# 001camellia/Speech-Imagery-EEG

Hardware: AMD Instinct MI355X
Metric: epochs/sec (B=256, C=122, T=1000) IGN 3-class (higher is better)
Workload: dtype f32

## Files before the change

speech-imagery-eeg_amd/csrc/ign_clconv_x6.hip:

```cpp
#include "ign_clconv.h"

typedef __bf16 bf16x8 __attribute__((ext_vector_type(8)));
constexpr int X6_PITCH = KC + 8;
constexpr int X6_PLANE = TM * X6_PITCH;
constexpr int X6_BLOCK = 3 * TN * KC;

typedef float f32x2 __attribute__((ext_vector_type(2)));
typedef __bf16 bf16x2 __attribute__((ext_vector_type(2)));
__device__ __forceinline__ void split3_pair(f32x2 v, bf16x2& x0, bf16x2& x1, bf16x2& x2) {
    x0 = __builtin_convertvector(v, bf16x2);
    f32x2 r = v - __builtin_convertvector(x0, f32x2);
    x1 = __builtin_convertvector(r, bf16x2);
    r -= __builtin_convertvector(x1, f32x2);
    x2 = __builtin_convertvector(r, bf16x2);
}
template <int V>
__device__ __forceinline__ void split3_store(const float (&t)[V], __bf16* d, int plane);
template <>
__device__ __forceinline__ void split3_store<1>(const float (&t)[1], __bf16* d, int plane);
__device__ __forceinline__ void split3(float v, __bf16& x0, __bf16& x1, __bf16& x2) {
    x0 = (__bf16)v;
    float r = v - (float)x0;
    x1 = (__bf16)r;
    r -= (float)x1;
    x2 = (__bf16)r;
}
template <>
__device__ __forceinline__ void split3_store<1>(const float (&t)[1], __bf16* d, int plane) {
    __bf16 x0, x1, x2;
    split3(t[0], x0, x1, x2);
    d[0] = x0; d[plane] = x1; d[2 * plane] = x2;
}
template <>
__device__ __forceinline__ void split3_store<2>(const float (&t)[2], __bf16* d, int plane) {
    bf16x2 x0, x1, x2;
    split3_pair(f32x2{t[0], t[1]}, x0, x1, x2);
    *reinterpret_cast<bf16x2*>(d) = x0;
    *reinterpret_cast<bf16x2*>(d + plane) = x1;
    *reinterpret_cast<bf16x2*>(d + 2 * plane) = x2;
}
template <>
__device__ __forceinline__ void split3_store<4>(const float (&t)[4], __bf16* d, int plane) {
    typedef __bf16 bf16x4 __attribute__((ext_vector_type(4)));
    bf16x2 a0, a1, a2, b0, b1, b2;
    split3_pair(f32x2{t[0], t[1]}, a0, a1, a2);
    split3_pair(f32x2{t[2], t[3]}, b0, b1, b2);
    *reinterpret_cast<bf16x4*>(d) = __builtin_shufflevector(a0, b0, 0, 1, 2, 3);
    *reinterpret_cast<bf16x4*>(d + plane) = __builtin_shufflevector(a1, b1, 0, 1, 2, 3);
    *reinterpret_cast<bf16x4*>(d + 2 * plane) = __builtin_shufflevector(a2, b2, 0, 1, 2, 3);
}

typedef _Float16 f16x2 __attribute__((ext_vector_type(2)));
typedef _Float16 f16x4 __attribute__((ext_vector_type(4)));
typedef _Float16 f16x8 __attribute__((ext_vector_type(8)));
__device__ __forceinline__ void split2h_pair(f32x2 v, f16x2& x0, f16x2& x1) {
    x0 = __builtin_convertvector(v, f16x2);
    x1 = __builtin_convertvector(v - __builtin_convertvector(x0, f32x2), f16x2);
}
template <int V>
__device__ __forceinline__ void split2h_store(const float (&t)[V], __bf16* d, int plane) {
    _Float16* dh = reinterpret_cast<_Float16*>(d);
    if constexpr (V == 1) {
        const _Float16 x0 = (_Float16)t[0];
        dh[0] = x0; dh[plane] = (_Float16)(t[0] - (float)x0);
    } else if constexpr (V == 2) {
        f16x2 x0, x1;
        split2h_pair(f32x2{t[0], t[1]}, x0, x1);
        *reinterpret_cast<f16x2*>(dh) = x0;
        *reinterpret_cast<f16x2*>(dh + plane) = x1;
    } else {
        f16x2 a0, a1, b0, b1;
        split2h_pair(f32x2{t[0], t[1]}, a0, a1);
        split2h_pair(f32x2{t[2], t[3]}, b0, b1);
        *reinterpret_cast<f16x4*>(dh) = __builtin_shufflevector(a0, b0, 0, 1, 2, 3);
        *reinterpret_cast<f16x4*>(dh + plane) = __builtin_shufflevector(a1, b1, 0, 1, 2, 3);
    }
}

template <int V, int NP>
__device__ __forceinline__ void split_store(const float (&t)[V], __bf16* d, int plane) {
    if constexpr (NP == 3) {
        split3_store<V>(t, d, plane);
    } else if constexpr (NP == 2) {
        split2h_store<V>(t, d, plane);
    } else if constexpr (V == 1) {
        d[0] = (__bf16)t[0];
    } else if constexpr (V == 2) {
        *reinterpret_cast<bf16x2*>(d) = __builtin_convertvector(f32x2{t[0], t[1]}, bf16x2);
    } else {
        typedef __bf16 bf16x4 __attribute__((ext_vector_type(4)));
        const bf16x2 a = __builtin_convertvector(f32x2{t[0], t[1]}, bf16x2), b = __builtin_convertvector(f32x2{t[2], t[3]}, bf16x2);
        *reinterpret_cast<bf16x4*>(d) = __builtin_shufflevector(a, b, 0, 1, 2, 3);
    }
}

template <int NP>
__device__ __forceinline__ f32x16 mfma16(const bf16x8& a, const bf16x8& b, const f32x16& c) {
    if constexpr (NP == 2)
        return __builtin_amdgcn_mfma_f32_32x32x16_f16(__builtin_bit_cast(f16x8, a), __builtin_bit_cast(f16x8, b), c, 0, 0, 0);
    else
        return __builtin_amdgcn_mfma_f32_32x32x16_bf16(a, b, c, 0, 0, 0);
}

#ifndef IGN_H3_WAVES
#define IGN_H3_WAVES 3
#endif
constexpr int X6T_SPAN = TM + 15;
constexpr int X6T_APLANE = X6T_SPAN * X6_PITCH;

template <int NP> struct X6tLds {
    static constexpr int NPL = (NP == 2) ? 2 : 3;
    static constexpr int ABUF = NPL * X6T_APLANE, BBUF = NPL * X6_PLANE;
    static constexpr size_t BYTES = (size_t)2 * (ABUF + BBUF) * sizeof(unsigned short);
};
template <int NP, int EPI> struct X6tWaves { static constexpr int N = (NP == 2 && EPI == EPI_BIAS_STATS) ? IGN_H3_WAVES : 2; };
template <int V, bool PRO, int EPI, int NP>
__global__ void __launch_bounds__(256, (X6tWaves<NP, EPI>::N)) clconv_x6t_kernel(const ConvX6Args ca) {
    const GemmNTArgs& a = ca.g;
    constexpr int VPR = KC / V;
    constexpr int APASS = (X6T_SPAN * VPR + 255) / 256;
    constexpr int X6T_ABUF = X6tLds<NP>::ABUF, X6T_BBUF = X6tLds<NP>::BBUF;
    extern __shared__ __attribute__((aligned(16))) unsigned short smem16[];
    __bf16* Abuf = reinterpret_cast<__bf16*>(smem16);
    __bf16* Bbuf = Abuf + 2 * X6T_ABUF;

    const int nwg = a.mtiles * a.ntiles;
    int lid = blockIdx.x;
    {
        const int per = nwg / 8;
        if (lid < per * 8) lid = (lid & 7) * per + (lid >> 3);
    }
    const int mt = lid / a.ntiles, nt = lid - mt * a.ntiles;
    const int bi = mt / ca.tps, tt = mt - bi * ca.tps;
    const int t0 = tt * TM, n0 = nt * TN;
    const int tid = threadIdx.x, lane = tid & 63, wave = tid >> 6;
    const int l31 = lane & 31, h = lane >> 5;
    const int wm = wave & 1, wn = wave >> 1;
    const int span = TM + ca.k - 1;
    const int nvec = span * VPR;

    const float* abase = a.A + (long long)bi * ca.sample_pitch;
    const int brw = tid >> 1, bh = tid & 1;
    const unsigned short* bsrc = a.B3 + (size_t)nt * (size_t)(ca.cp / KC) * ca.k * X6_BLOCK + (size_t)brw * KC + 8 * bh;
    constexpr size_t bplane = (size_t)TN * KC;

    f32x16 acc[2][2];
#pragma unroll
    for (int i = 0; i < 2; ++i)
#pragma unroll
        for (int j = 0; j < 2; ++j)
#pragma unroll
            for (int r = 0; r < 16; ++r) acc[i][j][r] = 0.f;

    float ra[APASS][V];
    float pa[V], pb[V];
    bool a_ok = false;
    uint4 rb00, rb01 = {}, rb02 = {}, rb10, rb11 = {}, rb12 = {};
    const int ncc = ca.cp / KC;
    const int nstep = ncc * ca.k;

    const float sa = (NP == 2) ? ign_pow2_scale(ca.bound_a) : 1.f;
    const float osc = (NP == 2) ? 1.f / (sa * ign_pow2_scale(ca.bound_b)) : 1.f;
    auto aload = [&](int cc) {
        const int ch = cc * KC + (tid % VPR) * V;
        a_ok = ch < ca.cin;
        if (PRO && a_ok) {
            vload<V>(pa, a.pro_a + ch); vload<V>(pb, a.pro_b + ch);
            if constexpr (NP == 2) {
#pragma unroll
                for (int v = 0; v < V; ++v) { pa[v] *= sa; pb[v] *= sa; }
            }
        }
#pragma unroll
        for (int p = 0; p < APASS; ++p) {
            const int idx = tid + p * 256;
            const int row = idx / VPR;
            if (a_ok && idx < nvec) vload<V>(ra[p], abase + (long long)min(t0 + row, ca.rows_in - 1) * ca.cin + ch);
            else {
#pragma unroll
                for (int v = 0; v < V; ++v) ra[p][v] = 0.f;
            }
        }
    };
    auto astore = [&](int buf) {
        __bf16* st = Abuf + buf * X6T_ABUF;
#pragma unroll
        for (int p = 0; p < APASS; ++p) {
            const int idx = tid + p * 256;
            if (idx < nvec) {
                const int row = idx / VPR, q = idx - row * VPR;
                float tv[V];
#pragma unroll
                for (int v = 0; v < V; ++v) {
                    tv[v] = ra[p][v];
                    if (PRO && a_ok) tv[v] = fmaxf(fmaf(pa[v], tv[v], pb[v]), 0.f);
                    else if (NP == 2) tv[v] *= sa;
                }
                split_store<V, NP>(tv, st + row * X6_PITCH + q * V, X6T_APLANE);
            }
        }
    };
    auto boff = [&](int st) {
        st = min(st, nstep - 1);
        return (size_t)st * X6_BLOCK;
    };
    auto bstore = [&](int buf, const uint4& r0, const uint4& r1, const uint4& r2) {
        __bf16* st = Bbuf + buf * X6T_BBUF + brw * X6_PITCH + 8 * bh;
        *reinterpret_cast<uint4*>(st) = r0;
        if constexpr (NP >= 2) *reinterpret_cast<uint4*>(st + X6_PLANE) = r1;
        if constexpr (NP == 3) *reinterpret_cast<uint4*>(st + 2 * X6_PLANE) = r2;
    };
#define IGN_BLOAD(r0, r1, r2, st)                                                                       \
    do {                                                                                                \
        const size_t off_ = boff(st);                                                                   \
        r0 = *reinterpret_cast<const uint4*>(bsrc + off_);                                              \
        if constexpr (NP >= 2) r1 = *reinterpret_cast<const uint4*>(bsrc + bplane + off_);              \
        if constexpr (NP == 3) r2 = *reinterpret_cast<const uint4*>(bsrc + 2 * bplane + off_);          \
    } while (0)

    aload(0);
    IGN_BLOAD(rb00, rb01, rb02, 0);
    IGN_BLOAD(rb10, rb11, rb12, 1);
    astore(0);
    bstore(0, rb00, rb01, rb02);
    __syncthreads();

    int cc = 0, j = 0;
    auto body = [&](int step, bool odd) {
        if (odd) IGN_BLOAD(rb10, rb11, rb12, step + 2);
        else IGN_BLOAD(rb00, rb01, rb02, step + 2);
        const bool next_span = cc + 1 < ncc;
        if (j == 0 && next_span) aload(cc + 1);
        const __bf16* As = Abuf + (cc & 1) * X6T_ABUF + (wm * 64 + l31 + j) * X6_PITCH + 8 * h;
        const __bf16* Bs = Bbuf + (step & 1) * X6T_BBUF + (wn * 64 + l31) * X6_PITCH + 8 * h;
        bf16x8 af[2][NP], bf[2][NP];
#pragma unroll
        for (int i = 0; i < 2; ++i)
#pragma unroll
            for (int pl = 0; pl < NP; ++pl) {
                af[i][pl] = *reinterpret_cast<const bf16x8*>(As + pl * X6T_APLANE + i * 32 * X6_PITCH);
                bf[i][pl] = *reinterpret_cast<const bf16x8*>(Bs + pl * X6_PLANE + i * 32 * X6_PITCH);
            }
        __builtin_amdgcn_sched_barrier(0);
#define IGN_X6(pa_, pb_)                                                                                   \
        acc[0][0] = mfma16<NP>(af[0][pa_], bf[0][pb_], acc[0][0]);                                         \
        acc[0][1] = mfma16<NP>(af[0][pa_], bf[1][pb_], acc[0][1]);                                         \
        acc[1][0] = mfma16<NP>(af[1][pa_], bf[0][pb_], acc[1][0]);                                         \
        acc[1][1] = mfma16<NP>(af[1][pa_], bf[1][pb_], acc[1][1]);
        if constexpr (NP == 3) { IGN_X6(2, 0) IGN_X6(0, 2) IGN_X6(1, 1) IGN_X6(1, 0) IGN_X6(0, 1) }
        if constexpr (NP == 2) { IGN_X6(1, 0) IGN_X6(0, 1) }
        IGN_X6(0, 0)
#undef IGN_X6
        __builtin_amdgcn_sched_barrier(0);
        if (odd) bstore((step + 1) & 1, rb00, rb01, rb02);
        else bstore((step + 1) & 1, rb10, rb11, rb12);
        if (j + 1 == ca.k) {
            if (next_span) astore((cc + 1) & 1);
            j = 0; ++cc;
        } else {
            ++j;
        }
        __syncthreads();
    };
    for (int step = 0; step < nstep; step += 2) {
        body(step, false);
        if (step + 1 < nstep) body(step + 1, true);
    }
#undef IGN_BLOAD
    const int m0 = bi * ca.trows + t0;
    nt_epilogue<EPI, NP == 2>(a, acc, reinterpret_cast<float*>(smem16), mt, m0, n0, bi * ca.trows + min(ca.trows, t0 + TM), osc);
}

#ifndef IGN_H3W_WAVES
#define IGN_H3W_WAVES 2
#endif
template <int NP> struct X6wLds {
    static constexpr int NPL = NP == 3 ? 3 : (NP == 2 ? 2 : 1);
    static constexpr int ABUF = NPL * TM * X6_PITCH;
    static constexpr int BBUF = 2 * NPL * X6_PLANE;
    static constexpr size_t BYTES = (size_t)2 * (ABUF + BBUF) * sizeof(unsigned short);
    static constexpr int WAVES = NP == 2 ? IGN_H3W_WAVES : 2;
};

template <int NP, int EPI = EPI_BIAS_STATS>
__global__ void __launch_bounds__(512, X6wLds<NP>::WAVES) clconv_x6w_kernel(const ConvX6Args ca) {
    const GemmNTArgs& a = ca.g;
    extern __shared__ __attribute__((aligned(16))) unsigned short smem16[];
    constexpr int X6W_ABUF = X6wLds<NP>::ABUF, X6W_BBUF = X6wLds<NP>::BBUF, NPL = X6wLds<NP>::NPL;
    __bf16* Abuf = reinterpret_cast<__bf16*>(smem16);
    __bf16* Bbuf = Abuf + 2 * X6W_ABUF;
    constexpr int APLANE = TM * X6_PITCH;

    const int ntw = a.N / 256;
    const int nwg = a.mtiles * ntw;
    int lid = blockIdx.x;
    {
        const int per = nwg / 8;
        if (lid < per * 8) lid = (lid & 7) * per + (lid >> 3);
    }
    const int mt = lid / ntw, nw = lid - mt * ntw;
    const int m0 = mt * TM, n0 = nw * 256;
    const int tid = threadIdx.x, lane = tid & 63, wave = tid >> 6;
    const int l31 = lane & 31, h = lane >> 5;
    const int wm = wave & 1, wn = wave >> 1;
    const int ncc = ca.cp / KC;

    f32x16 acc[2][2];
#pragma unroll
    for (int i = 0; i < 2; ++i)
#pragma unroll
        for (int j = 0; j < 2; ++j)
#pragma unroll
            for (int r = 0; r < 16; ++r) acc[i][j][r] = 0.f;

    const int arow = tid >> 2, ach = (tid & 3) * 4;
    const float* ap = a.A + (long long)min(m0 + arow, a.M - 1) * ca.cin + ach;
    float ra0[4], ra1[4];
    const int bt = tid >> 8, brw = (tid & 255) >> 1, bh = tid & 1;
    const unsigned short* bsrc = a.B3 + (size_t)(2 * nw + bt) * (size_t)ncc * X6_BLOCK + (size_t)brw * KC + 8 * bh;
    constexpr size_t bplane = (size_t)TN * KC;
    uint4 rb00, rb01 = {}, rb02 = {}, rb10, rb11 = {}, rb12 = {};

    const float sa = (NP == 2) ? ign_pow2_scale(ca.bound_a) : 1.f;
    const float osc = (NP == 2) ? 1.f / (sa * ign_pow2_scale(ca.bound_b)) : 1.f;
#define IGN_ALOADW(ra_, cc_)                                                                 \
    do {                                                                                     \
        const int c_ = min((cc_), ncc - 1);                                                  \
        if (c_ * KC + ach < ca.cin) vload<4>(ra_, ap + c_ * KC);           \
        else ra_[0] = ra_[1] = ra_[2] = ra_[3] = 0.f;                                        \
    } while (0)
    auto astore = [&](int buf, const float (&r)[4]) {
        if constexpr (NP == 2) {
            const float rs[4] = {r[0] * sa, r[1] * sa, r[2] * sa, r[3] * sa};
            split_store<4, NP>(rs, Abuf + buf * X6W_ABUF + arow * X6_PITCH + ach, APLANE);
        } else {
            split_store<4, NP>(r, Abuf + buf * X6W_ABUF + arow * X6_PITCH + ach, APLANE);
        }
    };
    auto bstore = [&](int buf, const uint4& r0, const uint4& r1, const uint4& r2) {
        __bf16* st = Bbuf + buf * X6W_BBUF + bt * NPL * X6_PLANE + brw * X6_PITCH + 8 * bh;
        *reinterpret_cast<uint4*>(st) = r0;
        if constexpr (NP >= 2) *reinterpret_cast<uint4*>(st + X6_PLANE) = r1;
        if constexpr (NP == 3) *reinterpret_cast<uint4*>(st + 2 * X6_PLANE) = r2;
    };
#define IGN_BLOADW(r0, r1, r2, st)                                                                      \
    do {                                                                                                \
        const size_t off_ = (size_t)min((st), ncc - 1) * X6_BLOCK;                                      \
        r0 = *reinterpret_cast<const uint4*>(bsrc + off_);                                              \
        if constexpr (NP >= 2) r1 = *reinterpret_cast<const uint4*>(bsrc + bplane + off_);              \
        if constexpr (NP == 3) r2 = *reinterpret_cast<const uint4*>(bsrc + 2 * bplane + off_);          \
    } while (0)

    IGN_ALOADW(ra0, 0);
    IGN_BLOADW(rb00, rb01, rb02, 0);
    IGN_ALOADW(ra1, 1);
    IGN_BLOADW(rb10, rb11, rb12, 1);
    astore(0, ra0);
    bstore(0, rb00, rb01, rb02);
    __syncthreads();

    const bool late = wave >= 4;
    auto mm = [&](int step) {
        const __bf16* As = Abuf + (step & 1) * X6W_ABUF + (wm * 64 + l31) * X6_PITCH + 8 * h;
        const __bf16* Bs = Bbuf + (step & 1) * X6W_BBUF + (wn >> 1) * NPL * X6_PLANE + ((wn & 1) * 64 + l31) * X6_PITCH + 8 * h;
        bf16x8 af[2][NP], bf[2][NP];
#pragma unroll
        for (int i = 0; i < 2; ++i)
#pragma unroll
            for (int pl = 0; pl < NP; ++pl) {
                af[i][pl] = *reinterpret_cast<const bf16x8*>(As + pl * APLANE + i * 32 * X6_PITCH);
                bf[i][pl] = *reinterpret_cast<const bf16x8*>(Bs + pl * X6_PLANE + i * 32 * X6_PITCH);
            }
        __builtin_amdgcn_sched_barrier(0);
#define IGN_X6(pa_, pb_)                                                                                   \
        acc[0][0] = mfma16<NP>(af[0][pa_], bf[0][pb_], acc[0][0]);                                         \
        acc[0][1] = mfma16<NP>(af[0][pa_], bf[1][pb_], acc[0][1]);                                         \
        acc[1][0] = mfma16<NP>(af[1][pa_], bf[0][pb_], acc[1][0]);                                         \
        acc[1][1] = mfma16<NP>(af[1][pa_], bf[1][pb_], acc[1][1]);
        if constexpr (NP == 3) { IGN_X6(2, 0) IGN_X6(0, 2) IGN_X6(1, 1) }
        if constexpr (NP >= 2) { IGN_X6(1, 0) IGN_X6(0, 1) }
        IGN_X6(0, 0)
#undef IGN_X6
        __builtin_amdgcn_sched_barrier(0);
    };
    auto body = [&](int step, bool odd) {
        if (odd) { IGN_BLOADW(rb10, rb11, rb12, step + 2); IGN_ALOADW(ra1, step + 2); }
        else { IGN_BLOADW(rb00, rb01, rb02, step + 2); IGN_ALOADW(ra0, step + 2); }
        const bool next = step + 1 < ncc;
        auto st = [&]() {
            if (odd) { bstore((step + 1) & 1, rb00, rb01, rb02); if (next) astore((step + 1) & 1, ra0); }
            else { bstore((step + 1) & 1, rb10, rb11, rb12); if (next) astore((step + 1) & 1, ra1); }
            __builtin_amdgcn_sched_barrier(0);
        };
        if (late) { st(); mm(step); } else { mm(step); st(); }
        __syncthreads();
    };
    for (int step = 0; step < ncc; step += 2) {
        body(step, false);
        if (step + 1 < ncc) body(step + 1, true);
    }
#undef IGN_BLOADW
#undef IGN_ALOADW
    float s1[2] = {0.f, 0.f}, s2[2] = {0.f, 0.f};
    const int m_lim = a.M;
    if (m0 + TM <= m_lim) nt_epilogue_body<EPI, true, NP == 2>(a, acc, s1, s2, m0, n0, m_lim, osc);
    else nt_epilogue_body<EPI, false, NP == 2>(a, acc, s1, s2, m0, n0, m_lim, osc);
}

__device__ __forceinline__ void pack_weights_x3t_body(const float* __restrict__ w, unsigned short* __restrict__ wt3,
                                                      unsigned short* __restrict__ wd3, int Co, int Ci, int k, int Cip, int Cop,
                                                      long long i, const float* __restrict__ bound = nullptr) {
    const long long nf = (long long)((Co + TN - 1) / TN) * (Cip / KC) * k * (TN * KC);
    const long long nd = wd3 ? (long long)((Ci + TN - 1) / TN) * (Cop / KC) * k * (TN * KC) : 0;
    const bool fwd = i < nf;
    if (!fwd && i >= nf + nd) return;
    const long long e = fwd ? i : i - nf;
    const int q = (int)(e % KC);
    long long t = e / KC;
    const int row = (int)(t % TN);
    t /= TN;
    const int j = (int)(t % k);
    t /= k;
    const int ncc = (fwd ? Cip : Cop) / KC;
// ... 214 lines not shown
    float* out = a.part + (long long)split * a.Co * a.k * a.Ci;
    const int ci = ci0 + wci * 32 + l31;
    if (ci < a.Ci) {
#pragma unroll
        for (int j = 0; j < KT; ++j)
#pragma unroll
            for (int r = 0; r < 16; ++r) {
                const int co = co0 + wco * 32 + acc_row16(r, h);
                if (co < a.Co) out[((long long)co * a.k + j) * a.Ci + ci] = (NP == 2) ? acc[j][r] * osc : acc[j][r];
            }
    }
}

constexpr int W1_PITCH = 128 + 32;
constexpr int W1_PLANE = 16 * W1_PITCH;

struct Wgrad1Args {
    const float* dy; const float* x; float* part;
    float* part_b;
    long long M;
    int Ci, Co, nunits, nsplit, citiles, ntiles;
    const float* bound_dy; const float* bound_x;
};

template <int NP>
__global__ void __launch_bounds__(256, (NP == 2 ? IGN_H3_WAVES : 2)) clconv_wgrad_x6_k1_kernel(const Wgrad1Args a) {
    extern __shared__ __attribute__((aligned(16))) unsigned short smem16[];
    __bf16* smem = reinterpret_cast<__bf16*>(smem16);
    constexpr int NPL = (NP == 2) ? 2 : 3;
    constexpr int W1_STAGE = 2 * NPL * W1_PLANE;
    const int xcd = blockIdx.x & 7, seq = blockIdx.x >> 3;
    const int tile = seq % a.ntiles;
    const int split = (seq / a.ntiles) * 8 + xcd;
    if (split >= a.nsplit) return;
    const int cot = tile / a.citiles, cit = tile - cot * a.citiles;
    const int co0 = cot * 128, ci0 = cit * 128;
    const int per = (a.nunits + a.nsplit - 1) / a.nsplit;
    const int u_begin = split * per, u_end = min(a.nunits, u_begin + per);

    const int tid = threadIdx.x, lane = tid & 63, wave = tid >> 6;
    const int l31 = lane & 31, h = lane >> 5;
    const int wco = wave & 1, wci = wave >> 1;

    const int sr = tid >> 5, sc = (tid & 31) * 4;
    const bool d_ok = co0 + sc < a.Co, x_ok = ci0 + sc < a.Ci;
    const float* dyp = a.dy + co0 + sc;
    const float* xp = a.x + ci0 + sc;

    f32x16 acc[2][2];
#pragma unroll
    for (int i = 0; i < 2; ++i)
#pragma unroll
        for (int j = 0; j < 2; ++j)
#pragma unroll
            for (int r = 0; r < 16; ++r) acc[i][j][r] = 0.f;

    float rd[2][4], rx[2][4];
    const float sdy = (NP == 2) ? ign_pow2_scale(a.bound_dy) : 1.f;
    const float sx = (NP == 2) ? ign_pow2_scale(a.bound_x) : 1.f;
    const float osc = (NP == 2) ? 1.f / (sdy * sx) : 1.f;
    const bool want_b = a.part_b != nullptr && cit == 0;
    float bsum[4] = {0.f, 0.f, 0.f, 0.f};
    auto gload = [&](int u) {
#pragma unroll
        for (int p = 0; p < 2; ++p) {
            const long long m = (long long)u * 16 + sr + 8 * p;
            if (d_ok && m < a.M) vload<4>(rd[p], dyp + m * a.Co);
            else { rd[p][0] = rd[p][1] = rd[p][2] = rd[p][3] = 0.f; }
            if (x_ok && m < a.M) vload<4>(rx[p], xp + m * a.Ci);
            else { rx[p][0] = rx[p][1] = rx[p][2] = rx[p][3] = 0.f; }
        }
    };
    auto lstore = [&](int buf) {
        __bf16* P = smem + buf * W1_STAGE;
        __bf16* Q = P + NPL * W1_PLANE;
        if (want_b) {
#pragma unroll
            for (int v = 0; v < 4; ++v) bsum[v] += rd[0][v] + rd[1][v];
        }
#pragma unroll
        for (int p = 0; p < 2; ++p) {
            if constexpr (NP == 2) {
#pragma unroll
                for (int v = 0; v < 4; ++v) { rd[p][v] *= sdy; rx[p][v] *= sx; }
            }
            split_store<4, NP>(rd[p], P + (sr + 8 * p) * W1_PITCH + sc, W1_PLANE);
            split_store<4, NP>(rx[p], Q + (sr + 8 * p) * W1_PITCH + sc, W1_PLANE);
        }
    };

    const int u16 = lane & 15, q4 = u16 >> 2, p4 = u16 & 3, G1 = (lane >> 4) & 1;
    const int roff = (8 * h + q4) * W1_PITCH + 16 * G1 + 4 * p4;

    if (u_begin < u_end) {
        gload(u_begin);
        lstore(0);
    }
    __syncthreads();
    int buf = 0;
    for (int u = u_begin; u < u_end; ++u, buf ^= 1) {
        if (u + 1 < u_end) gload(u + 1);
        const __bf16* P = smem + buf * W1_STAGE + roff + wco * 64;
        const __bf16* Q = smem + buf * W1_STAGE + NPL * W1_PLANE + roff + wci * 64;
        bf16x8 bf[2][NP], af[2][NP];
#pragma unroll
        for (int j = 0; j < 2; ++j)
#pragma unroll
            for (int pl = 0; pl < NP; ++pl) {
                bf[j][pl] = lds_tr8(Q + pl * W1_PLANE + 32 * j, Q + pl * W1_PLANE + 32 * j + 4 * W1_PITCH);
                af[j][pl] = lds_tr8(P + pl * W1_PLANE + 32 * j, P + pl * W1_PLANE + 32 * j + 4 * W1_PITCH);
            }
        __builtin_amdgcn_sched_barrier(0);
#define IGN_W1(pa_, pb_)                                                                                   \
        acc[0][0] = mfma16<NP>(af[0][pa_], bf[0][pb_], acc[0][0]);                                         \
        acc[0][1] = mfma16<NP>(af[0][pa_], bf[1][pb_], acc[0][1]);                                         \
        acc[1][0] = mfma16<NP>(af[1][pa_], bf[0][pb_], acc[1][0]);                                         \
        acc[1][1] = mfma16<NP>(af[1][pa_], bf[1][pb_], acc[1][1]);
        if constexpr (NP == 3) { IGN_W1(2, 0) IGN_W1(0, 2) IGN_W1(1, 1) }
        if constexpr (NP >= 2) { IGN_W1(1, 0) IGN_W1(0, 1) }
        IGN_W1(0, 0)
#undef IGN_W1
        __builtin_amdgcn_sched_barrier(0);
        if (u + 1 < u_end) lstore(buf ^ 1);
        __syncthreads();
    }

    if (want_b) {
        float* red = reinterpret_cast<float*>(smem16);
        *reinterpret_cast<float4*>(red + sr * 128 + sc) = make_float4(bsum[0], bsum[1], bsum[2], bsum[3]);
        __syncthreads();
        if (tid < 128 && co0 + tid < a.Co) {
            float t = 0.f;
#pragma unroll
            for (int r = 0; r < 8; ++r) t += red[r * 128 + tid];
            a.part_b[(long long)split * a.Co + co0 + tid] = t;
        }
    }
    float* out = a.part + (long long)split * a.Co * a.Ci;
#pragma unroll
    for (int j = 0; j < 2; ++j) {
        const int ci = ci0 + wci * 64 + 32 * j + l31;
        if (ci < a.Ci) {
#pragma unroll
            for (int i = 0; i < 2; ++i)
#pragma unroll
                for (int r = 0; r < 16; ++r) {
                    const int co = co0 + wco * 64 + 32 * i + acc_row16(r, h);
                    if (co < a.Co) out[(long long)co * a.Ci + ci] = (NP == 2) ? acc[i][j][r] * osc : acc[i][j][r];
                }
        }
    }
}

template <int EPI, int NP>
static int launch_x6t(const ConvX6Args& a, int V, bool pro, hipStream_t s) {
    const dim3 grid((unsigned)(a.g.mtiles * a.g.ntiles)), block(256);
#define IGN_X6T(VV, PP)                                                                                                      \
    do {                                                                                                                     \
        static bool once = false;                                                                                            \
        if (!once) {                                                                                                         \
            (void)hipFuncSetAttribute(reinterpret_cast<const void*>(&clconv_x6t_kernel<VV, PP, EPI, NP>),                     \
                                      hipFuncAttributeMaxDynamicSharedMemorySize, (int)X6tLds<NP>::BYTES);                   \
            once = true;                                                                                                     \
        }                                                                                                                    \
        hipLaunchKernelGGL((clconv_x6t_kernel<VV, PP, EPI, NP>), grid, block, X6tLds<NP>::BYTES, s, a);                       \
    } while (0)
    if constexpr (EPI == EPI_PLAIN) {
        if (pro) { ign_set_error("clconv_x6t_kernel: the plain epilogue has no prologue variant"); return IGN_E_UNSUP; }
        if (V == 4) IGN_X6T(4, false); else if (V == 2) IGN_X6T(2, false); else IGN_X6T(1, false);
    } else {
        if (V == 4) { if (pro) IGN_X6T(4, true); else IGN_X6T(4, false); }
        else if (V == 2) { if (pro) IGN_X6T(2, true); else IGN_X6T(2, false); }
        else { if (pro) IGN_X6T(1, true); else IGN_X6T(1, false); }
    }
#undef IGN_X6T
    return ign_check_launch("clconv_x6t_kernel");
}

template <int NP, int EPI = EPI_BIAS_STATS>
static int launch_x6w(const ConvX6Args& a, hipStream_t s) {
    static bool once = false;
    if (!once) {
        (void)hipFuncSetAttribute(reinterpret_cast<const void*>(&clconv_x6w_kernel<NP, EPI>), hipFuncAttributeMaxDynamicSharedMemorySize,
                                  (int)X6wLds<NP>::BYTES);
        once = true;
    }
    const unsigned nwg = (unsigned)(a.g.mtiles * (a.g.N / 256));
    hipLaunchKernelGGL((clconv_x6w_kernel<NP, EPI>), dim3(nwg), dim3(512), X6wLds<NP>::BYTES, s, a);
    return ign_check_launch("clconv_x6w_kernel");
}

int ign_clconv_launch_x6t(const ConvX6Args& a, int epi, int V, bool pro, hipStream_t s) {
    if (epi == EPI_GELU_BWD) {
        if (!(a.k == 1 && a.g.N % 256 == 0 && V == 4 && !pro && !a.g.part && a.tps * 1 == a.g.mtiles && a.trows == a.g.M && a.nprod == 3
              && a.g.ey)) {
            ign_set_error("ign_clconv_launch_x6t: the GELU-gradient epilogue needs k = 1, N %% 256 == 0, C %% 4 == 0, the f16x3 arithmetic");
            return IGN_E_UNSUP;
        }
        return launch_x6w<2, EPI_GELU_BWD>(a, s);
    }
    if (a.k == 1 && a.g.N % 256 == 0 && V == 4 && !pro && epi == EPI_BIAS_STATS && !a.g.part &&
        a.tps * 1 == a.g.mtiles && a.trows == a.g.M)
        return a.nprod == 1 ? launch_x6w<1>(a, s) : a.nprod == 3 ? launch_x6w<2>(a, s) : launch_x6w<3>(a, s);
    if (epi == EPI_PLAIN)
        return a.nprod == 1 ? launch_x6t<EPI_PLAIN, 1>(a, V, pro, s) : a.nprod == 3 ? launch_x6t<EPI_PLAIN, 2>(a, V, pro, s)
                                                                                      : launch_x6t<EPI_PLAIN, 3>(a, V, pro, s);
    if (a.nprod == 1)
        return epi == EPI_BIAS_STATS ? launch_x6t<EPI_BIAS_STATS, 1>(a, V, pro, s) : launch_x6t<EPI_MASK_STATS, 1>(a, V, pro, s);
    if (a.nprod == 3)
        return epi == EPI_BIAS_STATS ? launch_x6t<EPI_BIAS_STATS, 2>(a, V, pro, s) : launch_x6t<EPI_MASK_STATS, 2>(a, V, pro, s);
    return epi == EPI_BIAS_STATS ? launch_x6t<EPI_BIAS_STATS, 3>(a, V, pro, s) : launch_x6t<EPI_MASK_STATS, 3>(a, V, pro, s);
}

extern "C" int ign_clconv_kpad(int C) { return (C + 15) / 16 * 16; }
extern "C" long long ign_clconv_x3_elems(int rows, int chans, int k) {
    return 3LL * ((rows + TN - 1) / TN) * TN * k * ((chans + 15) / 16 * 16);
}
extern "C" long long ign_clconv_x6_mtiles(int B, int rows) { return (long long)B * ((rows + TM - 1) / TM); }

extern "C" int ign_clconv_pack_weights_x3(const float* w_oik, void* wt3_fwd, void* wt3_dgrad, int Co, int Ci, int k, void* stream) {
    if (!w_oik || !wt3_fwd || Co <= 0 || Ci <= 0 || k <= 0) {
        ign_set_error("ign_clconv_pack_weights_x3: bad argument (Co=%d Ci=%d k=%d)", Co, Ci, k);
        return IGN_E_ARG;
    }
    const int Cip = ign_clconv_kpad(Ci), Cop = ign_clconv_kpad(Co);
    const long long n = ign_clconv_x3_elems(Co, Ci, k) / 3 + (wt3_dgrad ? ign_clconv_x3_elems(Ci, Co, k) / 3 : 0);
    hipLaunchKernelGGL(pack_weights_x3t_kernel, dim3((unsigned)((n + 255) / 256)), dim3(256), 0, (hipStream_t)stream, w_oik,
                       (unsigned short*)wt3_fwd, (unsigned short*)wt3_dgrad, Co, Ci, k, Cip, Cop);
    return ign_check_launch("pack_weights_x3t_kernel");
}

static int pack_multi_impl(int n, const float* const* w_oik, void* const* wt3_fwd, void* const* wt3_dgrad, const int* Co, const int* Ci,
                           const int* k, long long* const* counters, const float* const* bounds, void* stream);

extern "C" int ign_clconv_pack_weights_x3_multi(int n, const float* const* w_oik, void* const* wt3_fwd, void* const* wt3_dgrad,
                                               const int* Co, const int* Ci, const int* k, long long* const* counters, void* stream) {
    return pack_multi_impl(n, w_oik, wt3_fwd, wt3_dgrad, Co, Ci, k, counters, nullptr, stream);
}

extern "C" int ign_clconv_pack_weights_h2_multi(int n, const float* const* w_oik, void* const* wt_fwd, void* const* wt_dgrad,
                                               const int* Co, const int* Ci, const int* k, long long* const* counters,
                                               const float* const* w_bounds, void* stream) {
    if (!w_bounds) { ign_set_error("ign_clconv_pack_weights_h2_multi: null bound table"); return IGN_E_ARG; }
    for (int l = 0; l < n && l < PACK_LMAX; ++l)
        if (!w_bounds[l]) { ign_set_error("ign_clconv_pack_weights_h2_multi: layer %d: null weight bound", l); return IGN_E_ARG; }
    return pack_multi_impl(n, w_oik, wt_fwd, wt_dgrad, Co, Ci, k, counters, w_bounds, stream);
}

static int pack_multi_impl(int n, const float* const* w_oik, void* const* wt3_fwd, void* const* wt3_dgrad, const int* Co, const int* Ci,
                           const int* k, long long* const* counters, const float* const* bounds, void* stream) {
    if (n <= 0 || n > PACK_LMAX || !w_oik || !wt3_fwd || !Co || !Ci || !k) {
        ign_set_error("ign_clconv_pack_weights_x3_multi: n=%d outside 1..%d or null table", n, PACK_LMAX);
        return IGN_E_ARG;
    }
    PackMultiTable t;
    long long nmax = 0;
    for (int l = 0; l < n; ++l) {
        if (!w_oik[l] || !wt3_fwd[l] || Co[l] <= 0 || Ci[l] <= 0 || k[l] <= 0) {
            ign_set_error("ign_clconv_pack_weights_x3_multi: layer %d: bad argument (Co=%d Ci=%d k=%d)", l, Co[l], Ci[l], k[l]);
            return IGN_E_ARG;
        }
        t.w[l] = w_oik[l]; t.wt3[l] = (unsigned short*)wt3_fwd[l]; t.wd3[l] = wt3_dgrad ? (unsigned short*)wt3_dgrad[l] : nullptr;
        t.counter[l] = counters ? counters[l] : nullptr;
        t.bound[l] = bounds ? bounds[l] : nullptr;
        t.Co[l] = Co[l]; t.Ci[l] = Ci[l]; t.k[l] = k[l];
        const long long e = ign_clconv_x3_elems(Co[l], Ci[l], k[l]) / 3 + (t.wd3[l] ? ign_clconv_x3_elems(Ci[l], Co[l], k[l]) / 3 : 0);
        nmax = e > nmax ? e : nmax;
    }
    hipLaunchKernelGGL(pack_weights_x3t_multi_kernel, dim3((unsigned)((nmax + 255) / 256), (unsigned)n), dim3(256), 0,
                       (hipStream_t)stream, t);
    return ign_check_launch("pack_weights_x3t_multi_kernel");
}

template <int KT, int NR, int NP>
static int launch_wgrad_x6(const WgradX6Args& a, int V, bool pro, dim3 grid, hipStream_t s) {
    constexpr size_t lds = (size_t)2 * (NP == 2 ? 2 : 3) * ((16 * NR) + (16 * NR + KT - 1)) * WG_PITCH * sizeof(unsigned short);
#define IGN_WG(VV, PP)                                                                                                       \
    do {                                                                                                                     \
        static bool once = false;                                                                                            \
        if (!once) {                                                                                                         \
            (void)hipFuncSetAttribute(reinterpret_cast<const void*>(&clconv_wgrad_x6_kernel<KT, NR, VV, PP, NP>),             \
                                      hipFuncAttributeMaxDynamicSharedMemorySize, (int)lds);                                 \
            once = true;                                                                                                     \
        }                                                                                                                    \
        hipLaunchKernelGGL((clconv_wgrad_x6_kernel<KT, NR, VV, PP, NP>), grid, dim3(256), lds, s, a);                         \
    } while (0)
    if (V == 4) { if (pro) IGN_WG(4, true); else IGN_WG(4, false); }
    else if (V == 2) { if (pro) IGN_WG(2, true); else IGN_WG(2, false); }
    else { if (pro) IGN_WG(1, true); else IGN_WG(1, false); }
#undef IGN_WG
    return ign_check_launch("clconv_wgrad_x6_kernel");
}

static int wgrad_x6_rows_per_unit(int k) { return (k == 8 || k == 5) ? 16 : (k == 3 || k == 2) ? 32 : 0; }
static int wgrad_x6_splits(int nunits, int tiles) {
    int s = (512 + tiles - 1) / tiles;
    const int max_s = (nunits + 15) / 16;
    if (s > max_s) s = max_s;
    return s < 1 ? 1 : s;
}

static int wgrad_x6_k1_splits(long long M, int Ci, int Co, int* nunits, int* tiles) {
    *nunits = (int)((M + 15) / 16);
    *tiles = ((Co + 127) / 128) * ((Ci + 127) / 128);
    int s = (512 + *tiles - 1) / *tiles;
    const int max_s = (*nunits + 31) / 32;
    if (s > max_s) s = max_s;
    return s < 1 ? 1 : s;
// ... 124 lines not shown
```

Measured before the change: 2.839.

## Add paired-step x6t conv kernel processing two k-steps per barrier for dgrad

Adds a new NP=2 conv kernel that handles two reduction steps per loop iteration, double-buffering a pair of B tiles in LDS and interleaving MFMA with LDS reads and writes through sched_group_barrier hints. It is meant to halve the __syncthreads count and hide LDS and global latency behind matrix work. By default it is enabled only for the mask-stats (dgrad) epilogue and can be toggled with an environment variable. It also drops the scheduling barriers around the MFMA block in the existing NP=2 path. The costs are higher register pressure, more LDS use and more complex chunk-staging logic.

```diff
diff --git a/speech-imagery-eeg_amd/csrc/ign_clconv_x6.hip b/speech-imagery-eeg_amd/csrc/ign_clconv_x6.hip
--- a/speech-imagery-eeg_amd/csrc/ign_clconv_x6.hip
+++ b/speech-imagery-eeg_amd/csrc/ign_clconv_x6.hip
@@ -1,4 +1,5 @@
 #include "ign_clconv.h"
+#include <cstdlib>
 
 typedef __bf16 bf16x8 __attribute__((ext_vector_type(8)));
 constexpr int X6_PITCH = KC + 8;
@@ -241,7 +242,7 @@
                 af[i][pl] = *reinterpret_cast<const bf16x8*>(As + pl * X6T_APLANE + i * 32 * X6_PITCH);
                 bf[i][pl] = *reinterpret_cast<const bf16x8*>(Bs + pl * X6_PLANE + i * 32 * X6_PITCH);
             }
-        __builtin_amdgcn_sched_barrier(0);
+        if constexpr (NP != 2) __builtin_amdgcn_sched_barrier(0);
 #define IGN_X6(pa_, pb_)                                                                                   \
         acc[0][0] = mfma16<NP>(af[0][pa_], bf[0][pb_], acc[0][0]);                                         \
         acc[0][1] = mfma16<NP>(af[0][pa_], bf[1][pb_], acc[0][1]);                                         \
@@ -251,7 +252,7 @@
         if constexpr (NP == 2) { IGN_X6(1, 0) IGN_X6(0, 1) }
         IGN_X6(0, 0)
 #undef IGN_X6
-        __builtin_amdgcn_sched_barrier(0);
+        if constexpr (NP != 2) __builtin_amdgcn_sched_barrier(0);
         if (odd) bstore((step + 1) & 1, rb00, rb01, rb02);
         else bstore((step + 1) & 1, rb10, rb11, rb12);
         if (j + 1 == ca.k) {
@@ -269,6 +270,201 @@
 #undef IGN_BLOAD
     const int m0 = bi * ca.trows + t0;
     nt_epilogue<EPI, NP == 2>(a, acc, reinterpret_cast<float*>(smem16), mt, m0, n0, bi * ca.trows + min(ca.trows, t0 + TM), osc);
+}
+
+constexpr bool X6T_PAIR_DEFAULT_FWD = false, X6T_PAIR_DEFAULT_DGRAD = true;
+struct X6tPairLds {
+    static constexpr int ABUF = 2 * X6T_APLANE, BBUF = 2 * X6_PLANE;
+    static constexpr size_t BYTES = (size_t)(2 * ABUF + 4 * BBUF) * sizeof(unsigned short);
+};
+template <int V, bool PRO, int EPI>
+__global__ void __launch_bounds__(256, 2) clconv_x6t_pair_kernel(const ConvX6Args ca) {
+    constexpr int NP = 2;
+    const GemmNTArgs& a = ca.g;
+    constexpr int VPR = KC / V;
+    constexpr int APASS = (X6T_SPAN * VPR + 255) / 256;
+    constexpr int X6T_ABUF = X6tPairLds::ABUF, X6T_BBUF = X6tPairLds::BBUF;
+    extern __shared__ __attribute__((aligned(16))) unsigned short smem16[];
+    __bf16* Abuf = reinterpret_cast<__bf16*>(smem16);
+    __bf16* Bbuf = Abuf + 2 * X6T_ABUF;
+
+    const int nwg = a.mtiles * a.ntiles;
+    int lid = blockIdx.x;
+    {
+        const int per = nwg / 8;
+        if (lid < per * 8) lid = (lid & 7) * per + (lid >> 3);
+    }
+    const int mt = lid / a.ntiles, nt = lid - mt * a.ntiles;
+    const int bi = mt / ca.tps, tt = mt - bi * ca.tps;
+    const int t0 = tt * TM, n0 = nt * TN;
+    const int tid = threadIdx.x, lane = tid & 63, wave = tid >> 6;
+    const int l31 = lane & 31, h = lane >> 5;
+    const int wm = wave & 1, wn = wave >> 1;
+    const int span = TM + ca.k - 1;
+    const int nvec = span * VPR;
+
+    const float* abase = a.A + (long long)bi * ca.sample_pitch;
+    const int brw = tid >> 1, bh = tid & 1;
+    const unsigned short* bsrc = a.B3 + (size_t)nt * (size_t)(ca.cp / KC) * ca.k * X6_BLOCK + (size_t)brw * KC + 8 * bh;
+    constexpr size_t bplane = (size_t)TN * KC;
+
+    f32x16 acc[2][2];
+#pragma unroll
+    for (int i = 0; i < 2; ++i)
+#pragma unroll
+        for (int j = 0; j < 2; ++j)
+#pragma unroll
+            for (int r = 0; r < 16; ++r) acc[i][j][r] = 0.f;
+
+    float ra[APASS][V];
+    float pa[V], pb[V];
+    bool a_ok = false;
+    uint4 rb00, rb01, rb02, rb03, rb10, rb11, rb12, rb13;
+    const int ncc = ca.cp / KC;
+    const int nstep = ncc * ca.k;
+
+    const float sa = ign_pow2_scale(ca.bound_a);
+    const float osc = 1.f / (sa * ign_pow2_scale(ca.bound_b));
+    auto aload = [&](int cc) {
+        const int ch = cc * KC + (tid % VPR) * V;
+        a_ok = ch < ca.cin;
+        if (PRO && a_ok) {
+            vload<V>(pa, a.pro_a + ch); vload<V>(pb, a.pro_b + ch);
+#pragma unroll
+            for (int v = 0; v < V; ++v) { pa[v] *= sa; pb[v] *= sa; }
+        }
+#pragma unroll
+        for (int p = 0; p < APASS; ++p) {
+            const int idx = tid + p * 256;
+            const int row = idx / VPR;
+            if (a_ok && idx < nvec) vload<V>(ra[p], abase + (long long)min(t0 + row, ca.rows_in - 1) * ca.cin + ch);
+            else {
+#pragma unroll
+                for (int v = 0; v < V; ++v) ra[p][v] = 0.f;
+            }
+        }
+    };
+    auto astore = [&](int buf) {
+        __bf16* st = Abuf + buf * X6T_ABUF;
+#pragma unroll
+        for (int p = 0; p < APASS; ++p) {
+            const int idx = tid + p * 256;
+            if (idx < nvec) {
+                const int row = idx / VPR, q = idx - row * VPR;
+                float tv[V];
+#pragma unroll
+                for (int v = 0; v < V; ++v) {
+                    tv[v] = ra[p][v];
+                    if (PRO && a_ok) tv[v] = fmaxf(fmaf(pa[v], tv[v], pb[v]), 0.f);
+                    else tv[v] *= sa;
+                }
+                split_store<V, NP>(tv, st + row * X6_PITCH + q * V, X6T_APLANE);
+            }
+        }
+    };
+    auto boff = [&](int st) {
+        st = min(st, nstep - 1);
+        return (size_t)st * X6_BLOCK;
+    };
+    auto bstore = [&](int par, const uint4& r0, const uint4& r1, const uint4& r2, const uint4& r3) {
+        __bf16* st = Bbuf + 2 * par * X6T_BBUF + brw * X6_PITCH + 8 * bh;
+        *reinterpret_cast<uint4*>(st) = r0;
+        *reinterpret_cast<uint4*>(st + X6_PLANE) = r1;
+        *reinterpret_cast<uint4*>(st + X6T_BBUF) = r2;
+        *reinterpret_cast<uint4*>(st + X6T_BBUF + X6_PLANE) = r3;
+    };
+#define IGN_BLOAD2(r0, r1, r2, r3, pr)                                                                  \
+    do {                                                                                                \
+        const size_t o0_ = boff(2 * (pr)), o1_ = boff(2 * (pr) + 1);                                    \
+        r0 = *reinterpret_cast<const uint4*>(bsrc + o0_);                                               \
+        r1 = *reinterpret_cast<const uint4*>(bsrc + bplane + o0_);                                      \
+        r2 = *reinterpret_cast<const uint4*>(bsrc + o1_);                                               \
+        r3 = *reinterpret_cast<const uint4*>(bsrc + bplane + o1_);                                      \
+    } while (0)
+#define IGN_X6(af_, bf_, pa_, pb_)                                                                         \
+    acc[0][0] = mfma16<NP>(af_[0][pa_], bf_[0][pb_], acc[0][0]);                                           \
+    acc[0][1] = mfma16<NP>(af_[0][pa_], bf_[1][pb_], acc[0][1]);                                           \
+    acc[1][0] = mfma16<NP>(af_[1][pa_], bf_[0][pb_], acc[1][0]);                                           \
+    acc[1][1] = mfma16<NP>(af_[1][pa_], bf_[1][pb_], acc[1][1]);
+
+    aload(0);
+    IGN_BLOAD2(rb00, rb01, rb02, rb03, 0);
+    IGN_BLOAD2(rb10, rb11, rb12, rb13, 1);
+    astore(0);
+    bstore(0, rb00, rb01, rb02, rb03);
+    __syncthreads();
+
+    int cc = 0, j = 0;
+    int cnext = 1, snext = ca.k;
+    bool staged = false;
+    const int lrow = wm * 64 + l31, brow = (wn * 64 + l31) * X6_PITCH + 8 * h;
+    auto body = [&](int p, bool odd) {
+        if (odd) IGN_BLOAD2(rb10, rb11, rb12, rb13, p + 2);
+        else IGN_BLOAD2(rb00, rb01, rb02, rb03, p + 2);
+        if (!staged && cnext < ncc) { aload(cnext); staged = true; }
+        const bool wrap = j + 1 == ca.k;
+        const int c1 = wrap ? cc + 1 : cc, j1 = wrap ? 0 : j + 1;
+        const __bf16* As0 = Abuf + (cc & 1) * X6T_ABUF + (lrow + j) * X6_PITCH + 8 * h;
+        const __bf16* As1 = Abuf + (c1 & 1) * X6T_ABUF + (lrow + j1) * X6_PITCH + 8 * h;
+        const __bf16* Bs = Bbuf + (odd ? 2 : 0) * X6T_BBUF + brow;
+        bf16x8 af0[2][NP], bf0[2][NP], af1[2][NP], bf1[2][NP];
+#pragma unroll
+        for (int i = 0; i < 2; ++i)
+#pragma unroll
+            for (int pl = 0; pl < NP; ++pl) {
+                af0[i][pl] = *reinterpret_cast<const bf16x8*>(As0 + pl * X6T_APLANE + i * 32 * X6_PITCH);
+                bf0[i][pl] = *reinterpret_cast<const bf16x8*>(Bs + pl * X6_PLANE + i * 32 * X6_PITCH);
+            }
+#pragma unroll
+        for (int i = 0; i < 2; ++i)
+#pragma unroll
+            for (int pl = 0; pl < NP; ++pl) {
+                af1[i][pl] = *reinterpret_cast<const bf16x8*>(As1 + pl * X6T_APLANE + i * 32 * X6_PITCH);
+                bf1[i][pl] = *reinterpret_cast<const bf16x8*>(Bs + X6T_BBUF + pl * X6_PLANE + i * 32 * X6_PITCH);
+            }
+        __builtin_amdgcn_sched_group_barrier(0x100, 8, 0);
+        __builtin_amdgcn_sched_group_barrier(0x008, 4, 0);
+        __builtin_amdgcn_sched_group_barrier(0x100, 4, 0);
+        __builtin_amdgcn_sched_group_barrier(0x008, 8, 0);
+        __builtin_amdgcn_sched_group_barrier(0x100, 4, 0);
+        __builtin_amdgcn_sched_group_barrier(0x008, 4, 0);
+        __builtin_amdgcn_sched_group_barrier(0x200, 4, 0);
+        __builtin_amdgcn_sched_group_barrier(0x008, 8, 0);
+        IGN_X6(af0, bf0, 1, 0) IGN_X6(af0, bf0, 0, 1) IGN_X6(af0, bf0, 0, 0)
+        if (odd) bstore(0, rb00, rb01, rb02, rb03);
+        else bstore(1, rb10, rb11, rb12, rb13);
+        IGN_X6(af1, bf1, 1, 0) IGN_X6(af1, bf1, 0, 1) IGN_X6(af1, bf1, 0, 0)
+        if (staged && (snext >> 1) == p + 1) {
+            astore(cnext & 1);
+            staged = false; ++cnext; snext += ca.k;
+        }
+        cc = c1; j = j1;
+        if (j + 1 == ca.k) { j = 0; ++cc; } else ++j;
+        __syncthreads();
+    };
+    const int nfull = nstep >> 1;
+    for (int p = 0; p < nfull; p += 2) {
+        body(p, false);
+        if (p + 1 < nfull) body(p + 1, true);
+    }
+    if (nstep & 1) {
+        const __bf16* As0 = Abuf + (cc & 1) * X6T_ABUF + (lrow + j) * X6_PITCH + 8 * h;
+        const __bf16* Bs = Bbuf + 2 * (nfull & 1) * X6T_BBUF + brow;
+        bf16x8 af0[2][NP], bf0[2][NP];
+#pragma unroll
+        for (int i = 0; i < 2; ++i)
+#pragma unroll
+            for (int pl = 0; pl < NP; ++pl) {
+                af0[i][pl] = *reinterpret_cast<const bf16x8*>(As0 + pl * X6T_APLANE + i * 32 * X6_PITCH);
+                bf0[i][pl] = *reinterpret_cast<const bf16x8*>(Bs + pl * X6_PLANE + i * 32 * X6_PITCH);
+            }
+        IGN_X6(af0, bf0, 1, 0) IGN_X6(af0, bf0, 0, 1) IGN_X6(af0, bf0, 0, 0)
+        __syncthreads();
+    }
+#undef IGN_X6
+#undef IGN_BLOAD2
+    const int m0 = bi * ca.trows + t0;
+    nt_epilogue<EPI, true>(a, acc, reinterpret_cast<float*>(smem16), mt, m0, n0, bi * ca.trows + min(ca.trows, t0 + TM), osc);
 }
 
 #ifndef IGN_H3W_WAVES
@@ -789,8 +985,47 @@
     }
 }
 
+static int x6t_pair_switch() {
+    static const int v = [] {
+        const char* e = std::getenv("IGN_X6T_PAIR");
+        return (e && *e) ? (std::atoi(e) != 0 ? 1 : 0) : -1;
+    }();
+    return v;
+}
+template <int EPI> struct X6tPairDefault { static constexpr bool ON = X6T_PAIR_DEFAULT_DGRAD && EPI == EPI_MASK_STATS; };
+template <> struct X6tPairDefault<EPI_BIAS_STATS> { static constexpr bool ON = X6T_PAIR_DEFAULT_FWD; };
+
+template <int EPI>
+static int launch_x6t_pair(const ConvX6Args& a, int V, bool pro, hipStream_t s) {
+    const dim3 grid((unsigned)(a.g.mtiles * a.g.ntiles)), block(256);
+#define IGN_X6TP(VV, PP)                                                                                                     \
+    do {                                                                                                                     \
+        static bool once = false;                                                                                            \
+        if (!once) {                                                                                                         \
+            (void)hipFuncSetAttribute(reinterpret_cast<const void*>(&clconv_x6t_pair_kernel<VV, PP, EPI>),                    \
+                                      hipFuncAttributeMaxDynamicSharedMemorySize, (int)X6tPairLds::BYTES);                   \
+            once = true;                                                                                                     \
+        }                                                                                                                    \
+        hipLaunchKernelGGL((clconv_x6t_pair_kernel<VV, PP, EPI>), grid, block, X6tPairLds::BYTES, s, a);                      \
+    } while (0)
+    if constexpr (EPI == EPI_PLAIN) {
+        if (V == 4) IGN_X6TP(4, false); else if (V == 2) IGN_X6TP(2, false); else IGN_X6TP(1, false);
+    } else {
+        if (V == 4) { if (pro) IGN_X6TP(4, true); else IGN_X6TP(4, false); }
+        else if (V == 2) { if (pro) IGN_X6TP(2, true); else IGN_X6TP(2, false); }
+        else { if (pro) IGN_X6TP(1, true); else IGN_X6TP(1, false); }
+    }
+#undef IGN_X6TP
+    return ign_check_launch("clconv_x6t_pair_kernel");
+}
+
 template <int EPI, int NP>
 static int launch_x6t(const ConvX6Args& a, int V, bool pro, hipStream_t s) {
+    if constexpr (NP == 2) {
+        const int sw = x6t_pair_switch();
+        if ((sw < 0 ? X6tPairDefault<EPI>::ON : sw == 1) && (a.k >= 2 || a.cp == KC) && !(EPI == EPI_PLAIN && pro))
+            return launch_x6t_pair<EPI>(a, V, pro, s);
+    }
     const dim3 grid((unsigned)(a.g.mtiles * a.g.ntiles)), block(256);
 #define IGN_X6T(VV, PP)                                                                                                      \
     do {                                                                                                                     \
```

After: 2.837. Within noise of the previous version (-0.1%).
